# 1pathplanningzzj/pointnet_refine

Measured on AMD Instinct MI355X. Metric: lane segments/sec (fwd+bwd) at B=4096,N=1024; HBM GB/s vs roofline, higher is better.
Workload: dtype f32 (large GEMMs: 2xfp16-split MFMA, 3 products, fp32 accumulate); 1 GPU; LineRefineNet training step (fwd + deep-supervision L1 + bwd + Adam), B=4096/GPU, N=1024, M=32, C=4; global_batch=4096, points=1024, parallelism=dp1, decoder_chunk=4096

## Files before the change

include/pointnet_refine_hip.h:

```cpp
#ifndef POINTNET_REFINE_HIP_H
#define POINTNET_REFINE_HIP_H

#include <stddef.h>
#include <stdint.h>

#ifdef __cplusplus
extern "C" {
#endif

#define PRH_OK 0
#define PRH_ERR_ARG (-1)
#define PRH_ERR_WORKSPACE (-2)
#define PRH_ERR_HIP (-3)

#define PRH_MAX_LAYERS 8

typedef struct {
  const float* w;
  const float* b;
  const float* gamma;
  const float* beta;
  float* running_mean;
  float* running_var;
  int64_t* num_batches_tracked;
// ... 396 lines not shown
                         int device, void* stream);

int prh_set_gemm_mode(int mode);
int prh_get_gemm_mode(void);

int prh_set_dropout_seed_source(const unsigned* device_word);

int prh_test_gemm_nt(const float* a, const float* w, float* c, int m, int n, int k,
                     void* workspace, size_t workspace_bytes, int device, void* stream);
size_t prh_test_gemm_tn_workspace_bytes(int p, int mo, int ni);
size_t prh_test_gate_backward_workspace_bytes(int out_dim);
int prh_test_gate_backward(const float* ctx, int B, int N, int in_channel, int out_dim, const float* gate_w1,
                           const float* gate_b1, const float* gate_w2, const float* gate_b2, const float* z_fus,
                           const float* bn_scale, const float* bn_shift, float* d_fused, float* gate, int recompute,
                           float* ws_a, float* ws_b, void* workspace, size_t workspace_bytes, int device, void* stream);
int prh_test_gemm_tn(const float* a, const float* b, float* c, float* colsum, int p, int mo,
                     int ni, void* workspace, size_t workspace_bytes, int device, void* stream);
size_t prh_test_gemm_tn_side_workspace_bytes(int p, int mo, int ni);
int prh_test_gemm_tn_side(const float* a, const float* b, float* c, float* colsum, int p, int mo,
                          int ni, float* dy, long lddy, const float* z, long ldz, const float* ka,
                          const float* kb, const float* kc, long rows, int cols, int side,
                          float* amax_out, void* workspace, size_t workspace_bytes, int device,
                          void* stream);

enum {
  PRH_REDUCE_SLABS = 0, PRH_REDUCE_BN_STAGE1 = 1, PRH_REDUCE_PARTIALS = 2, PRH_REDUCE_LN_PARAM_GRAD = 3,
  PRH_REDUCE_FINAL = 4, PRH_REDUCE_ACT_AMAX = 5
};
int prh_test_reduce_depth(int kind);
int prh_test_reduce_slabs(const float* slab, int s, int rows, int cols, float* out, long ldout,
// ... 32 lines not shown
```

pointnet_refine_amd/_lib.py:

```python
from __future__ import annotations

import ctypes as C
import os
import subprocess
import threading

_HERE = os.path.dirname(os.path.abspath(__file__))
_ROOT = os.path.dirname(_HERE)
LIB_PATH = os.environ.get("PRH_LIB_PATH") or os.path.join(_HERE, "libpointnet_refine_hip.so")
_CSRC = os.path.join(_HERE, "csrc")
_SOURCES = [os.path.join(_CSRC, "prh_lib.hip")] + (sorted(
    os.path.join(_CSRC, f) for f in os.listdir(_CSRC) if f.endswith((".hpp", ".h", ".hip")) and f != "prh_lib.hip")
    if os.path.isdir(_CSRC) else [])
_HEADER = os.path.join(_ROOT, "include", "pointnet_refine_hip.h")

PRH_MAX_LAYERS = 8


class BnLayer(C.Structure):
    _fields_ = [("w", C.c_void_p), ("b", C.c_void_p), ("gamma", C.c_void_p), ("beta", C.c_void_p),
                ("running_mean", C.c_void_p), ("running_var", C.c_void_p),
                ("num_batches_tracked", C.c_void_p), ("cin", C.c_int), ("cout", C.c_int)]


# ... 30 lines not shown
    "prh_encoder_bf16_workspace_bytes", "prh_encoder_forward_bf16", "prh_encoder_backward_bf16",
    "prh_linear_bf16_workspace_bytes", "prh_linear_forward_bf16", "prh_linear_backward_bf16",
    "prh_linear_forward_out16", "prh_linear_backward_dy16", "prh_attn_forward_kv16", "prh_attn_backward_kv16",
    "prh_encoder_fused_image_bytes", "prh_encoder_fused_prepare", "prh_encoder_fused_workspace_bytes",
    "prh_encoder_fused_forward",
    "prh_linear_forward_workspace_bytes", "prh_linear_forward", "prh_linear_forward_ex",
    "prh_linear_forward_full", "prh_linear_forward_amax", "prh_operand_absmax_workspace_bytes", "prh_operand_absmax",
    "prh_linear_uses_operand_maxima", "prh_linear_backward_full", "prh_linear_backward_amax", "prh_pos_hidden_forward",
    "prh_pos_hidden_forward_workspace_bytes", "prh_pos_hidden_forward_amax", "prh_pos_hidden_backward_workspace_bytes",
    "prh_pos_hidden_backward", "prh_linear_small_forward", "prh_linear_small_backward_workspace_bytes",
    "prh_linear_small_backward",
    "prh_linear_backward_workspace_bytes", "prh_linear_backward", "prh_linear_backward_ex",
    "prh_mlp_stack_workspace_bytes", "prh_mlp_stack_forward", "prh_mlp_stack_backward",
    "prh_test_gemm_nt", "prh_test_gemm_tn_workspace_bytes", "prh_test_gemm_tn",
    "prh_test_gate_backward_workspace_bytes", "prh_test_gate_backward",
    "prh_test_gemm_tn_side_workspace_bytes", "prh_test_gemm_tn_side", "prh_test_xcc_map",
    "prh_test_reduce_depth", "prh_test_reduce_slabs", "prh_test_reduce_bn_stage1", "prh_test_reduce_partials",
    "prh_test_reduce_ln_param_grad", "prh_test_reduce_pos_hidden_final", "prh_test_reduce_partial_rows_final",
    "prh_test_reduce_act_amax_workspace_bytes", "prh_test_reduce_act_amax",
    "prh_profile_enable", "prh_profile_count", "prh_profile_reset", "prh_profile_read",
    "prh_attn_forward", "prh_attn_backward", "prh_attn_backward_ex",
    "prh_context_workspace_bytes", "prh_context_build",
    "prh_context_ragged_workspace_bytes", "prh_context_ragged_count", "prh_context_ragged_select",
    "prh_line_metrics", "prh_shift_sweep_workspace_bytes", "prh_shift_sweep",
    "prh_shift_sweep_ragged_workspace_bytes", "prh_shift_sweep_ragged",
    "prh_drive_slice_workspace_bytes", "prh_drive_slice_count", "prh_drive_slice_write",
    "prh_drive_clip_workspace_bytes", "prh_drive_clip_count", "prh_drive_clip_write",
    "prh_drive_noise_workspace_bytes", "prh_drive_noise",
    "prh_match_clip_workspace_bytes", "prh_match_clip_count", "prh_match_clip_write",
    "prh_match_costs_workspace_bytes", "prh_match_costs", "prh_match_max_side", "prh_match_assign",
# ... 329 lines not shown
    lib.prh_set_dropout_seed_source.argtypes = [vp]
    lib.prh_get_gemm_mode.restype = i
    lib.prh_profile_enable.restype = i
    lib.prh_profile_enable.argtypes = [i]
    lib.prh_profile_count.restype = i
    lib.prh_profile_reset.restype = i
    lib.prh_profile_read.restype = i
    lib.prh_profile_read.argtypes = [i, C.c_char_p, i, C.POINTER(C.c_float), C.POINTER(C.c_double),
                                     C.POINTER(C.c_double)]
    lib.prh_test_gemm_nt.restype = i
    lib.prh_test_gemm_nt.argtypes = [vp, vp, vp, i, i, i, vp, sz, i, vp]
    lib.prh_test_gate_backward_workspace_bytes.restype = sz
    lib.prh_test_gate_backward_workspace_bytes.argtypes = [i]
    lib.prh_test_gate_backward.restype = i
    lib.prh_test_gate_backward.argtypes = [vp, i, i, i, i, vp, vp, vp, vp, vp, vp, vp, vp, vp, i, vp, vp, vp, sz, i, vp]
    lib.prh_test_gemm_tn_workspace_bytes.restype = sz
    lib.prh_test_gemm_tn_workspace_bytes.argtypes = [i, i, i]
    lib.prh_test_gemm_tn.restype = i
    lib.prh_test_gemm_tn.argtypes = [vp, vp, vp, vp, i, i, i, vp, sz, i, vp]
    lib.prh_test_gemm_tn_side_workspace_bytes.restype = sz
    lib.prh_test_gemm_tn_side_workspace_bytes.argtypes = [i, i, i]
    lib.prh_test_gemm_tn_side.restype = i
    lib.prh_test_gemm_tn_side.argtypes = [vp, vp, vp, vp, i, i, i, vp, lg, vp, lg, vp, vp, vp, lg, i, i, vp, vp, sz, i, vp]
    lib.prh_test_xcc_map.restype = i
    lib.prh_test_xcc_map.argtypes = [i, i, vp, i, vp]
    if not hasattr(lib, "prh_test_reduce_depth"):
        return lib
    lib.prh_test_reduce_depth.restype = i
    lib.prh_test_reduce_depth.argtypes = [i]
    lib.prh_test_reduce_slabs.restype = i
# ... 38 lines not shown
```

pointnet_refine_amd/csrc/prh_gemm.hpp:

```cpp
#pragma once
#include <hip/hip_runtime.h>
#include <type_traits>
#include <stdint.h>

namespace prh {

typedef float f32x16 __attribute__((ext_vector_type(16)));

enum { PRO_NONE = 0, PRO_BNRELU = 1, PRO_BNBWD = 2, PRO_GATE1 = 3 };
enum { EPI_BIAS = 0, EPI_BIAS_STATS = 1, EPI_GATE = 2, EPI_DGRAD = 3, EPI_GATE_BWD = 4 };

enum {
  F_RELU_OUT = 1,
  F_ACCUM = 2,
  F_MASK = 4,
  F_STATS = 8,
  F_STORE_GATE = 16,
  F_E1_ROWVEC = 32,
  F_RESID = 64,
  F_DROPOUT = 256,
  F_POOL = 128,
};

struct NTParams {
  const float* A;  long lda;
  const float* A2; long lda2;
  const float* W;  long ldw;
  float* C;        long ldc;
  int M, N, K;
  const float* bias;
  const float* pa; const float* pb; const float* pc;
  const float* E1; long lde1;
  const float* es; const float* et;
  float* C2;       long ldc2;
  float* ws_a; float* ws_b;
  float* ws_c; float* ws_d;
  int flags;
  int tiles_n;
  char* wprep;
  const float* amaxA;
  const float* amaxW;
  unsigned drop_seed, drop_thresh;
  float drop_scale;
  const unsigned* seed_src;
};

__device__ __forceinline__ bool epi_keep(unsigned seed, unsigned row, unsigned col, unsigned thresh) {
  unsigned x = seed ^ (row * 0x9E3779B1u) ^ (col * 0x85EBCA77u);
  x ^= x >> 16; x *= 0x85EBCA6Bu; x ^= x >> 13; x *= 0xC2B2AE35u; x ^= x >> 16;
  return x >= thresh;
}
__device__ __forceinline__ unsigned epi_seed(const NTParams& p) {
  if (p.seed_src == nullptr) return p.drop_seed;
  const unsigned w = __hip_atomic_load(p.seed_src, __ATOMIC_RELAXED, __HIP_MEMORY_SCOPE_AGENT);
  return p.drop_seed ^ (__builtin_amdgcn_readfirstlane(w) * 0x9E3779B9u);
}

constexpr int BM = 128, BN = 128, BK = 32;

// ... 316 lines not shown
template <bool H>
__device__ __forceinline__ void st4e(char* base, int off, float4 v) {
  if (H) *reinterpret_cast<uint2*>(base + (size_t)off * 2) = make_uint2(pack_bf16x2(v.x, v.y), pack_bf16x2(v.z, v.w));
  else *reinterpret_cast<float4*>(base + (size_t)off * 4) = v;
}

typedef char* __restrict__ epi_wptr_r;
typedef const char* __restrict__ epi_rptr_r;
template <int EPI, int MT, class ACC, bool C16, bool AMAX = false>
__device__ __forceinline__ void nt_epilogue_vec_r2(ACC& acc, const NTParams& p, int rbase_,
                                                int cbase, int rb, int lane, float* scratch,
                                                bool bias_done = false,
                                                float* wave_amax = nullptr,
                                                float* zscr = nullptr) {
  static_assert(!AMAX || (EPI == EPI_BIAS && !C16), "output maximum: EPI_BIAS with fp32 storage");
  static_assert(EPI != EPI_GATE_BWD || !C16, "gate backward: fp32 storage");
  typedef typename std::conditional<AMAX || EPI == EPI_GATE_BWD, char*, epi_wptr_r>::type wptr;
  typedef typename std::conditional<AMAX || EPI == EPI_GATE_BWD, const char*, epi_rptr_r>::type rptr;
  const int rbase = __builtin_amdgcn_readfirstlane(rbase_);
  const float* biasp = bias_done ? nullptr : p.bias;
  constexpr int ES = C16 ? 2 : 4;
  const bool rowvec = EPI == EPI_DGRAD && (p.flags & F_E1_ROWVEC) != 0;
  const int ees = (C16 && !rowvec) ? 2 : 4;
  wptr Cb = reinterpret_cast<char*>(p.C) + (size_t)rbase * p.ldc * ES;
  rptr Eb = p.E1 != nullptr ? reinterpret_cast<const char*>(p.E1) + (size_t)rbase * p.lde1 * ees : nullptr;
  const int ldc = (int)p.ldc, lde1 = (int)p.lde1;
  const int mrows = p.M - rbase;
  const int rr = lane >> 4, c4 = (lane & 15) * 4;
  const int col4 = cbase + c4;
  const bool c4ok = col4 < p.N;
  float4 bias4 = zero4(), es4 = zero4(), et4 = zero4();
  if (c4ok) {
    if (biasp != nullptr) bias4 = ldg4(biasp + col4);
    if ((EPI == EPI_DGRAD && (p.flags & F_MASK) != 0) || EPI == EPI_GATE || EPI == EPI_GATE_BWD) {
      es4 = ldg4(p.es + col4);
      et4 = ldg4(p.et + col4);
    }
  }
  char* __restrict__ C2b = ((EPI == EPI_GATE || EPI == EPI_GATE_BWD) && p.C2 != nullptr) ? reinterpret_cast<char*>(p.C2) + (size_t)rbase * p.ldc2 * ES : nullptr;
  const int ldc2 = (int)p.ldc2;

  if (EPI == EPI_BIAS_STATS) epi_col_stats(acc, p, cbase, mrows, rb, lane, biasp);

  const bool mask = (p.flags & F_MASK) != 0, accum = (p.flags & F_ACCUM) != 0;
  const bool stats = EPI == EPI_DGRAD && (p.flags & F_STATS) != 0;
  const bool resid = EPI == EPI_BIAS && (p.flags & F_RESID) != 0;
  const unsigned dseed = (EPI == EPI_BIAS && (p.flags & F_DROPOUT) != 0) ? epi_seed(p) : 0u;
  const bool need_z = (EPI == EPI_DGRAD && (mask || stats)) || EPI == EPI_GATE || EPI == EPI_GATE_BWD || resid;
  float4 s1 = zero4(), s2 = zero4();
  const bool pool = EPI == EPI_GATE && (p.flags & F_POOL) != 0;
  float pmx[4] = {-1.f, -1.f, -1.f, -1.f}, psm[4] = {0.f, 0.f, 0.f, 0.f};
  int pix[4] = {0, 0, 0, 0};
  const int col4c = col4 < p.N ? col4 : (p.N - 4);
  rptr Cl = mrows > 0 ? Cb : reinterpret_cast<const char*>(p.C);
  rptr El = mrows > 0 ? Eb : reinterpret_cast<const char*>(p.E1);
  const bool acc_old = (EPI == EPI_DGRAD && accum) || EPI == EPI_GATE_BWD;
  float amx = 0.f;
  float t1 = 0.f, t2 = 0.f;
  constexpr int NB = 2 * MT;
  float4 zz[2][4], oo[2][4];
  auto issue = [&](int b, float4 (&z)[4], float4 (&o)[4]) {
    const char* Em = El; const char* Cm = Cl;
    asm volatile("" : "+s"(Em), "+s"(Cm) : : "memory");
    int lrc[4];
#pragma unroll
    for (int i = 0; i < 4; ++i) {
      z[i] = zero4(); o[i] = zero4();
      int r = (b >> 1) * 32 + ((b & 1) * 4 + i) * 4 + rr;
      r = r < mrows ? r : mrows - 1;
      lrc[i] = r < 0 ? 0 : r;
    }
// ... 57 lines not shown
          for (int e = 0; e < 4; ++e) {
            if (vv[e] > pmx[e]) { pmx[e] = vv[e]; pix[e] = lr; }
            psm[e] += vv[e];
          }
        }
      } else if (EPI == EPI_GATE_BWD) {
        const float4 m = gate_m4(v);
        float4 dg;
        gate_bwd_elem(o.x, z.x, m.x, es4.x, et4.x, v.x, dg.x);
        gate_bwd_elem(o.y, z.y, m.y, es4.y, et4.y, v.y, dg.y);
        gate_bwd_elem(o.z, z.z, m.z, es4.z, et4.z, v.z, dg.z);
        gate_bwd_elem(o.w, z.w, m.w, es4.w, et4.w, v.w, dg.w);
        if (ok) st4e<C16>(C2b, lr * ldc2 + col4, dg);
        *reinterpret_cast<float4*>(scratch + lrow * EPI_LDW + c4) = v;
        *reinterpret_cast<float4*>(zscr + (i * 4 + rr) * EPI_LDW + c4) = z;
      } else {
        if (resid) { v.x += z.x; v.y += z.y; v.z += z.z; v.w += z.w; }
        if ((p.flags & F_RELU_OUT) != 0) {
          v.x = fmaxf(v.x, 0.f); v.y = fmaxf(v.y, 0.f); v.z = fmaxf(v.z, 0.f); v.w = fmaxf(v.w, 0.f);
        }
        if (EPI == EPI_BIAS && (p.flags & F_DROPOUT) != 0) {
          const unsigned rw = (unsigned)(rbase + lr), c0 = (unsigned)col4;
          v.x = epi_keep(dseed, rw, c0, p.drop_thresh) ? v.x * p.drop_scale : 0.f;
          v.y = epi_keep(dseed, rw, c0 + 1, p.drop_thresh) ? v.y * p.drop_scale : 0.f;
          v.z = epi_keep(dseed, rw, c0 + 2, p.drop_thresh) ? v.z * p.drop_scale : 0.f;
          v.w = epi_keep(dseed, rw, c0 + 3, p.drop_thresh) ? v.w * p.drop_scale : 0.f;
        }
      }
      if (ok) st4e<C16>(Cb, lr * ldc + col4, v);
      if (AMAX && ok) amx = fmaxf(fmaxf(amx, fmaxf(fabsf(v.x), fabsf(v.y))), fmaxf(fabsf(v.z), fabsf(v.w)));
    }
    if (EPI == EPI_DGRAD)
      asm volatile("" : "+v"(s1.x), "+v"(s1.y), "+v"(s1.z), "+v"(s1.w), "+v"(s2.x), "+v"(s2.y), "+v"(s2.z), "+v"(s2.w));
    if constexpr (EPI == EPI_GATE_BWD) {
      const int nv = mrows - (mt * 32 + hb * 16);
      float c1 = 0.f, c2 = 0.f;
      if (nv >= 16) {
#pragma unroll
        for (int j = 0; j < 16; ++j) {
          const float dyj = scratch[(hb * 16 + j) * EPI_LDW + lane];
          c1 += dyj;
          c2 = fmaf(dyj, zscr[j * EPI_LDW + lane], c2);
        }
      } else {
        int nvv = nv;
// ... 31 lines not shown
      *reinterpret_cast<float4*>(p.ws_a + (size_t)rb * p.N + col4) = make_float4(pmx[0], pmx[1], pmx[2], pmx[3]);
      *reinterpret_cast<float4*>(p.ws_b + (size_t)rb * p.N + col4) = make_float4(psm[0], psm[1], psm[2], psm[3]);
      *reinterpret_cast<int4*>(p.ws_c + (size_t)rb * p.N + col4) = make_int4(pix[0], pix[1], pix[2], pix[3]);
    }
  }
  if (stats) {
    s1.x += __shfl_xor(s1.x, 16); s1.y += __shfl_xor(s1.y, 16); s1.z += __shfl_xor(s1.z, 16); s1.w += __shfl_xor(s1.w, 16);
    s2.x += __shfl_xor(s2.x, 16); s2.y += __shfl_xor(s2.y, 16); s2.z += __shfl_xor(s2.z, 16); s2.w += __shfl_xor(s2.w, 16);
    s1.x += __shfl_xor(s1.x, 32); s1.y += __shfl_xor(s1.y, 32); s1.z += __shfl_xor(s1.z, 32); s1.w += __shfl_xor(s1.w, 32);
    s2.x += __shfl_xor(s2.x, 32); s2.y += __shfl_xor(s2.y, 32); s2.z += __shfl_xor(s2.z, 32); s2.w += __shfl_xor(s2.w, 32);
    if (lane < 16 && c4ok) {
      *reinterpret_cast<float4*>(p.ws_a + (size_t)rb * p.N + col4) = s1;
      *reinterpret_cast<float4*>(p.ws_b + (size_t)rb * p.N + col4) = s2;
    }
  }
  if (AMAX) {
#pragma unroll
    for (int o = 32; o > 0; o >>= 1) amx = fmaxf(amx, __shfl_xor(amx, o));
    *wave_amax = amx;
  }
}

template <int EPI, int MT, class ACC, bool C16 = false, bool AMAX = false>
__device__ __forceinline__ void nt_epilogue_vec(ACC& acc, const NTParams& p, int rbase_,
                                                int cbase, int rb, int lane, float* scratch,
                                                bool bias_done = false,
                                                float* wave_amax = nullptr,
                                                float* zscr = nullptr) {
  if constexpr (!C16) {
    nt_epilogue_vec_r2<EPI, MT, ACC, false, AMAX>(acc, p, rbase_, cbase, rb, lane, scratch, bias_done, wave_amax, zscr);
    return;
  }
  static_assert(EPI != EPI_GATE_BWD || !C16, "gate backward: fp32 storage");
  const int rbase = __builtin_amdgcn_readfirstlane(rbase_);
  const float* biasp = bias_done ? nullptr : p.bias;
  constexpr int ES = C16 ? 2 : 4;
  const bool rowvec = EPI == EPI_DGRAD && (p.flags & F_E1_ROWVEC) != 0;
  const int ees = (C16 && !rowvec) ? 2 : 4;
  char* __restrict__ Cb = reinterpret_cast<char*>(p.C) + (size_t)rbase * p.ldc * ES;
  const char* __restrict__ Eb = p.E1 != nullptr ? reinterpret_cast<const char*>(p.E1) + (size_t)rbase * p.lde1 * ees : nullptr;
  const int ldc = (int)p.ldc, lde1 = (int)p.lde1;
  const int mrows = p.M - rbase;
  const int rr = lane >> 4, c4 = (lane & 15) * 4;
  const int col4 = cbase + c4;
  const bool c4ok = col4 < p.N;
  float4 bias4 = zero4(), es4 = zero4(), et4 = zero4();
  if (c4ok) {
    if (biasp != nullptr) bias4 = ldg4(biasp + col4);
// ... 424 lines not shown
```

pointnet_refine_amd/csrc/prh_gemm_h2.hpp:

```cpp
#pragma once
#include "prh_gemm_s3.hpp"

namespace prh {

constexpr int H2_BK = 32;
constexpr int H2_PLANE = 256 * H2_BK * 2;
constexpr int H2_OPER = 2 * H2_PLANE;
constexpr int H2_STAGE = 2 * H2_OPER;
constexpr int H2_LDS = 2 * H2_STAGE;

__device__ __forceinline__ int h2_off(int row, int k) {
  return row * 64 + ((((k >> 3) ^ (-(row >> 2))) & 3) << 4) + ((k & 7) << 1);
}

inline size_t h2_weight_bytes(int N, int K) {
  return S3_WHDR + (size_t)((N + 255) / 256) * ((K + H2_BK - 1) / H2_BK) * H2_OPER;
}

__global__ __launch_bounds__(256) void prep_weights_h2_kernel(const float* __restrict__ W, int N,
                                                              int K, long ldw, char* __restrict__ out,
                                                              const float* __restrict__ amax) {
  const int KT = (K + H2_BK - 1) / H2_BK;
  const int NT_ = (N + 255) / 256;
  const long total = (long)NT_ * 256 * KT * 4;
// ... 278 lines not shown
      tile(kt + 1, std::integral_constant<int, 0>{}, std::false_type{});
    }
    if (kt < KT) tile(kt, std::integral_constant<int, 1>{}, std::true_type{});
    if (kt + 1 < KT) tile(kt + 1, std::integral_constant<int, 0>{}, std::true_type{});
    if (wr == 0) __builtin_amdgcn_s_barrier();
  }
  asm volatile("s_waitcnt vmcnt(0)" ::: "memory");
  __syncthreads();
  PRH_TICK(1)
#pragma unroll
  for (int i = 0; i < 8; ++i)
#pragma unroll
    for (int j = 0; j < 4; ++j)
#pragma unroll
      for (int r = 0; r < 4; ++r) acc[i][j][r] *= unscale;
  if constexpr (AMAX) {
    float wmax = 0.f;
    nt_epilogue_vec<EPI, 4, f32x4[8][4], false, true>(acc, p, m0 + wm, n0 + wn, tile_m * 2 + (wave >> 2), lane,
                                                       reinterpret_cast<float*>(smem) + wave * (32 * EPI_LDW), false, &wmax);
    __syncthreads();
    float* red = reinterpret_cast<float*>(smem);
    if (lane == 0) red[wave] = wmax;
    __syncthreads();
    if (tid == 0)
      p.ws_a[blockIdx.x] = fmaxf(fmaxf(fmaxf(red[0], red[1]), fmaxf(red[2], red[3])),
                                 fmaxf(fmaxf(red[4], red[5]), fmaxf(red[6], red[7])));
  } else if constexpr (EPI == EPI_GATE_BWD) {
    static_assert(8 * (32 + 16) * EPI_LDW * 4 <= H2_LDS, "gate-backward scratch must fit in the stage buffers");
    nt_epilogue_vec<EPI, 4>(acc, p, m0 + wm, n0 + wn, tile_m * 2 + (wave >> 2), lane,
                            reinterpret_cast<float*>(smem) + wave * (32 * EPI_LDW), false, nullptr,
                            reinterpret_cast<float*>(smem) + 8 * (32 * EPI_LDW) + wave * (16 * EPI_LDW));
  } else {
    nt_epilogue_vec<EPI, 4>(acc, p, m0 + wm, n0 + wn, tile_m * 2 + (wave >> 2), lane,
// ... 309 lines not shown
```

pointnet_refine_amd/csrc/prh_lib.hip:

```cpp
#include "../../include/pointnet_refine_hip.h"

#include <hip/hip_runtime.h>
#include <stdarg.h>
#include <stdio.h>
#include <string.h>

#include <mutex>
#include <vector>

#include <stdlib.h>

#include "prh_gemm.hpp"
#include "prh_attn.hpp"
#include "prh_attn16.hpp"
#include "prh_gemm_s3.hpp"
#include "prh_gemm_h2.hpp"
#include "prh_b16.hpp"
#include "prh_small.hpp"
#include "prh_attnfold.hpp"
#include "prh_fused.hpp"
#include "prh_context.hpp"
#include "prh_metrics.hpp"
#include "prh_drive.hpp"
#include "prh_match.hpp"
// ... 385 lines not shown
}
template <int PRO, int EPI>
int launch_nt_core(Cores c, NTParams& p, hipStream_t st, StatInfo* si, float* amax_part, long* amax_tiles) {
  if (p.M <= 0 || p.N <= 0) return PRH_OK;
  if ((p.K & 3) || (PRO != PRO_GATE1 && (p.lda & 3)) || (p.ldw & 3) ||
      (PRO == PRO_BNBWD && (p.lda2 & 3)))
    return fail(PRH_ERR_ARG, "gemm_nt: K/lda/ldw must be multiples of 4 (K=%d lda=%ld ldw=%ld)",
                p.K, p.lda, p.ldw);
  if constexpr (PRO == PRO_NONE && EPI == EPI_BIAS) {
    if (c.mode == 4 && c.core == 2 && nt_b16_generic_ok(p)) return launch_nt_b16<PRO_NONE, EPI_BIAS, false, false>(p, st, si);
  }
  const bool want_pool = (p.flags & F_POOL) != 0;
  p.flags &= ~F_POOL;
  char nm[64];
  const double by = 4.0 * ((double)p.M * p.K * (PRO == PRO_BNBWD ? 2 : (PRO == PRO_GATE1 ? 0 : 1)) +
                           (double)p.M * p.N * (EPI == EPI_GATE_BWD ? 4 : (EPI == EPI_GATE ? 3 : (EPI == EPI_DGRAD ? 2 : 1))) +
                           (double)p.N * p.K);
  {
    if (p.wprep != nullptr && nt_use_s3(c, p.M, p.N, p.K) && p.lda <= 65536 && p.lda2 <= 65536 &&
        !((EPI == EPI_GATE || EPI == EPI_GATE_BWD) && ((p.N | (int)p.ldc | (int)p.lde1 | (int)p.ldc2) & 3) != 0)) {
      const int KT = cdiv(p.K, S3_BK), NTl = cdiv(p.N, S3_BN);
      const long th = (long)NTl * 256 * KT * 2;
      float* hdr = reinterpret_cast<float*>(p.wprep);
      const char* img = p.wprep + S3_WHDR;
      if (c.core == 3) {
        if (p.amaxW == nullptr) {
          TRY_RC((measure_absmax<PRO_NONE>(p.W, p.ldw, nullptr, 0, nullptr, nullptr, nullptr, p.N, p.K, hdr, hdr + 64, st)));
          p.amaxW = hdr;
        }
        if (p.amaxA == nullptr) {
          TRY_RC((measure_absmax<PRO>(p.A, p.lda, p.A2, p.lda2, p.pa, p.pb, p.pc, p.M, p.K, hdr + 1, hdr + 64, st)));
          p.amaxA = hdr + 1;
        }
      }
      if constexpr (PRO == PRO_NONE || PRO == PRO_BNRELU || PRO == PRO_GATE1) {
// ... 23 lines not shown
              *amax_tiles = wgs;
              return PRH_OK;
            }
          }
          if (g_h2_pp)
            hipLaunchKernelGGL((gemm_nt_h2_kernel<PRO, EPI, true>), dim3((unsigned)(NTl * cdiv(p.M, 256))), dim3(512),
                               lds, st, p, img);
          else
            hipLaunchKernelGGL((gemm_nt_h2_kernel<PRO, EPI>), dim3((unsigned)(NTl * cdiv(p.M, 256))), dim3(512),
                               lds, st, p, img);
          LAUNCH_CHECK();
          if (si) { si->count = 2 * cdiv(p.M, S3_BM); si->rows = 128; }
          return PRH_OK;
        }
      }
      if constexpr (EPI != EPI_GATE_BWD) {
        hipLaunchKernelGGL(prep_weights_s3_kernel, dim3((unsigned)cdiv(th, 256)), dim3(256), 0, st,
                           p.W, p.N, p.K, p.ldw, 0, p.wprep + S3_WHDR, c.core == 3 ? p.amaxW : nullptr);
        LAUNCH_CHECK();
        p.tiles_n = NTl;
        const long tiles = (long)NTl * cdiv(p.M, S3_BM);
        static const int attr_rc = allow_big_lds(gemm_nt_s3_kernel<PRO, EPI, 3>, gemm_nt_s3_kernel<PRO, EPI, 1>,
                                                 gemm_nt_s3_kernel<PRO, EPI, 2>);
        if (attr_rc != PRH_OK) return attr_rc;
        snprintf(nm, sizeof(nm), "gemm_nt_%s<%d,%d> K=%d N=%d", c.core == 3 ? "h2g1" : c.tag(), PRO, EPI, p.K, p.N);
        ProfScope ps(nm, 2.0 * p.M * (double)p.N * p.K, by, st);
        switch (c.core) {
          case 2: launch_nt_s3<PRO, EPI, 1>(p, tiles, img, st); break;
          case 3: launch_nt_s3<PRO, EPI, 2>(p, tiles, img, st); break;
          default: launch_nt_s3<PRO, EPI, 3>(p, tiles, img, st);
        }
        LAUNCH_CHECK();
        if (si) { si->count = 2 * cdiv(p.M, S3_BM); si->rows = 128; }
        return PRH_OK;
      }
    }
  }
  if constexpr (EPI == EPI_GATE_BWD) {
    return fail(PRH_ERR_ARG, "gemm_nt: the gate-recompute backward needs the split-fp16 core (M=%d N=%d)", p.M, p.N);
  } else {
    if constexpr (PRO == PRO_NONE && EPI == EPI_BIAS) {
      if (small_nt_ok(p, false)) return launch_small<false>(p, st);
    }
    p.tiles_n = cdiv(p.N, BN);
    const long tiles = (long)p.tiles_n * cdiv(p.M, BM);
    snprintf(nm, sizeof(nm), "gemm_nt<%d,%d> K=%d N=%d", PRO, EPI, p.K, p.N);
    ProfScope ps(nm, 2.0 * p.M * (double)p.N * p.K, by, st);
    if (p.N <= 64)
      hipLaunchKernelGGL((gemm_nt_kernel<PRO, EPI, true>), dim3((unsigned)tiles), dim3(256), 0, st, p);
    else
      hipLaunchKernelGGL((gemm_nt_kernel<PRO, EPI>), dim3((unsigned)tiles), dim3(256), 0, st, p);
    LAUNCH_CHECK();
    if (si) { si->count = 2 * cdiv(p.M, BM); si->rows = 64; }
// ... 991 lines not shown
  const int P = B * N;
  if (!recompute) {
    hipLaunchKernelGGL(combine_bwd_kernel, dim3(cdiv(P, 64), cdiv(od, 64)), dim3(256), 0, st, d_fused, d_gfeat,
                       argmax, z_fus, gate, es, et, P, N, od, dyf, ws_a, ws_b);
    LAUNCH_CHECK();
    return PRH_OK;
  }
  if (dyf != d_fused)
    HIP_TRY(hipMemcpyAsync(dyf, d_fused, (size_t)P * od * sizeof(float), hipMemcpyDeviceToDevice, st));
  NTParams p; memset(&p, 0, sizeof(p));
  p.A = inten; p.lda = C; p.pa = gate_w1; p.pb = gate_b1;
  p.W = gate_w2; p.ldw = 64; p.K = 64; p.M = P; p.N = od; p.bias = gate_b2;
  p.E1 = z_fus; p.lde1 = od; p.es = es; p.et = et;
  p.C = dyf; p.ldc = od; p.C2 = gate; p.ldc2 = od;
  p.ws_a = ws_a; p.ws_b = ws_b; p.wprep = wprep;
  return launch_nt<PRO_GATE1, EPI_GATE_BWD>(c, p, st);
}

int prh_encoder_gate_recompute(int B, int N, int in_channel, int out_dim, int want_global) {
  if (B <= 0 || N <= 0 || in_channel < 4 || out_dim <= 0 || (long)B * N > 2000000000L) return 0;
  return (!want_global && gate_on_h2(cores_of(gemm_mode()), B * N, out_dim, in_channel)) ? 1 : 0;
}

int prh_encoder_forward(const prh_encoder_params* prm, const float* ctx, int B, int N,
                        int training, float momentum, float eps, float* fused, float* gfeat,
                        const prh_encoder_saved* sv, void* workspace, size_t workspace_bytes,
                        int device, void* stream) {
  TRY(check_encoder(prm));
  if (!ctx || !fused || !sv || !sv->z_cat || !sv->z_fus || !sv->bn_scale || !sv->bn_shift ||
      !sv->bn_mean || !sv->bn_rstd || B <= 0 || N <= 0)
    return fail(PRH_ERR_ARG, "encoder_forward: bad argument");
// ... 79 lines not shown
  enc_carve(c, a, ews, P, prm->conv, cat, od, d_fused_scratch ? 2 : 1);
  StackWS& w = ews.w;
  StackBwdScratch& sc = ews.sc;
  float *fslab = ews.fslab, *fcslab = ews.fcslab, *dy_cat = ews.dy_cat, *dU = ews.dU, *dyf = d_fused_scratch ? d_fused : ews.dyf;
  float *gsum_a = ews.gsum_a, *gsum_b = ews.gsum_b;
  if (!a.ok) return fail(PRH_ERR_WORKSPACE, "encoder_backward: workspace too small (%zu bytes)", workspace_bytes);
  StackDims d = stack_dims(prm->conv, 5);
  if (d.cin0p != d.cin0) {
    TRY(copy_cols(ctx, d.cin0, d.cin0, w.xpad, d.cin0p, d.cin0p, (size_t)P, st));
    TRY(copy_cols(prm->conv[0].w, d.cin0, d.cin0, w.w0pad, d.cin0p, d.cin0p, (size_t)prm->conv[0].cout, st));
  }

  if (sv->gate_recompute && (d_gfeat != nullptr || !gate_on_h2(c, P, od, C)))
    return fail(PRH_ERR_ARG, "encoder_backward: saved.gate_recompute without prh_encoder_gate_recompute() "
                             "(pooled gradient, GEMM mode or shape)");
  TRY(gate_combine_backward(c, ctx + 3, C, B, N, od, prm->gate_w1, prm->gate_b1, prm->gate_w2, prm->gate_b2, sv->z_fus,
                            sv->bn_scale + cat, sv->bn_shift + cat, d_fused, d_gfeat, sv->argmax, sv->gate,
                            sv->gate_recompute, dyf, w.ws_a, w.ws_b, w.wprep, st));
  TRY(reduce_bn_stage1(w.ws_a, w.ws_b, cdiv(P, 64), (long)od, od, 64, P, 0, w.stat2, st));
  hipLaunchKernelGGL(bn_bwd_finalize_kernel, dim3(cdiv(od, 128)), dim3(128), 0, st, w.stat2, P, od,
                     prm->fusion.gamma, sv->bn_mean + cat, sv->bn_rstd + cat,
                     training, sc.ca, sc.cb, sc.cc, gr->fusion.dgamma, gr->fusion.dbeta,
                     gr->fusion.db);
  LAUNCH_CHECK();
  float* dG = sv->gate;

  StatInfo si5;
  const float* dzf_amax = nullptr;
  const bool matf = dz_in_place(c, od, (long)od, (long)od);
  if (matf) {
    TRY(materialize_dz(dyf, (long)od, sv->z_fus, (long)od, sc.ca, sc.cb, sc.cc, P, od, sc.hdr[0], st));
    dzf_amax = sc.hdr[0];
  }
  HeldWgrad hf;
  if (gr->fusion.dw) {
    TNParams t; memset(&t, 0, sizeof(t));
    t.A = dyf; t.lda = od; t.A2 = sv->z_fus; t.lda2 = od; t.pa = sc.ca; t.pb = sc.cb; t.pc = sc.cc;
    t.B = sv->z_cat; t.ldb = cat; t.qa = sv->bn_scale; t.qb = sv->bn_shift;
    t.P = P; t.Mo = od; t.Ni = cat;
    t.amaxA = dzf_amax;
    if (training && c.mode == 3 && sv->op_amax != nullptr) t.amaxB = sv->op_amax + 5;
    if (matf && dz_in_place(c, od, (long)cat, (long)cat) &&
        tn_side_ok(c, t, side_job(dy_cat + d.off[4], (long)cat, sv->z_cat + d.off[4], (long)cat, sc, P, od, sc.hdr[1]))) {
      hf.on = true; hf.t = t; hf.slab = fslab; hf.colslab = fcslab; hf.out = gr->fusion.dw; hf.ldc = (long)cat;
    } else if (matf) TRY((launch_tn<PRO_NONE, PRO_BNRELU>(c, t, fslab, fcslab, gr->fusion.dw, (long)cat, nullptr, st)));
// ... 1965 lines not shown
  p.A = a; p.lda = k; p.W = w; p.ldw = k; p.C = c; p.ldc = n; p.M = m; p.N = n; p.K = k;
  if (workspace != nullptr && workspace_bytes >= s3_weight_bytes(n, k) + 256)
    p.wprep = (char*)(((uintptr_t)workspace + 255) & ~(uintptr_t)255);
  return launch_nt<PRO_NONE, EPI_BIAS>(cores_of(gemm_mode()), p, (hipStream_t)stream);
}
size_t prh_test_gate_backward_workspace_bytes(int out_dim) { return s3_weight_bytes(out_dim, 64) + 512; }
int prh_test_gate_backward(const float* ctx, int B, int N, int in_channel, int out_dim, const float* gate_w1,
                           const float* gate_b1, const float* gate_w2, const float* gate_b2, const float* z_fus,
                           const float* bn_scale, const float* bn_shift, float* d_fused, float* gate, int recompute,
                           float* ws_a, float* ws_b, void* workspace, size_t workspace_bytes, int device, void* stream) {
  HIP_TRY(hipSetDevice(device));
  if (!ctx || !gate_w1 || !gate_b1 || !gate_w2 || !gate_b2 || !z_fus || !bn_scale || !bn_shift || !d_fused || !gate ||
      !ws_a || !ws_b || B <= 0 || N <= 0 || in_channel < 4 || out_dim <= 0 || (long)B * N > 2000000000L)
    return fail(PRH_ERR_ARG, "test_gate_backward: bad argument");
  const Cores c = cores_of(gemm_mode());
  if (recompute && !gate_on_h2(c, B * N, out_dim, in_channel))
    return fail(PRH_ERR_ARG, "test_gate_backward: recompute without prh_encoder_gate_recompute()");
  if (workspace == nullptr || workspace_bytes < prh_test_gate_backward_workspace_bytes(out_dim))
    return fail(PRH_ERR_WORKSPACE, "test_gate_backward: workspace too small");
  char* wprep = (char*)(((uintptr_t)workspace + 255) & ~(uintptr_t)255);
  return gate_combine_backward(c, ctx + 3, in_channel, B, N, out_dim, gate_w1, gate_b1, gate_w2, gate_b2, z_fus, bn_scale,
                               bn_shift, d_fused, nullptr, nullptr, gate, recompute, d_fused, ws_a, ws_b, wprep,
                               (hipStream_t)stream);
}
int prh_test_xcc_map(int blocks, int lds_bytes, int* out, int device, void* stream) {
  HIP_TRY(hipSetDevice(device));
  if (blocks <= 0 || lds_bytes < 0 || lds_bytes > 160 * 1024 || out == nullptr)
    return fail(PRH_ERR_ARG, "test_xcc_map: bad arguments");
  static const int attr_rc = allow_big_lds(xcc_probe_kernel);
  if (attr_rc != PRH_OK) return attr_rc;
  hipLaunchKernelGGL(xcc_probe_kernel, dim3((unsigned)blocks), dim3(512), (size_t)lds_bytes,
                     (hipStream_t)stream, out);
  LAUNCH_CHECK();
  return PRH_OK;
}
size_t prh_test_gemm_tn_workspace_bytes(int p, int mo, int ni) {
  const Cores c = cores_of(gemm_mode());
  Arena a;
// ... 119 lines not shown
```

pointnet_refine_amd/ops.py:

```python
from __future__ import annotations

import ctypes as C
import math
import threading
import weakref
from typing import List, Optional, Sequence

import torch

from . import _lib as L

_workspaces = {}


def _ws(device: torch.device, nbytes: int) -> torch.Tensor:
    key = (device.index, torch.cuda.current_stream(device).cuda_stream)
    t = _workspaces.get(key)
    if t is None or t.numel() < nbytes:
        _workspaces.pop(key, None)
        t = None
        t = torch.empty(int(nbytes * 1.05) + 4096, dtype=torch.uint8, device=device)
        _workspaces[key] = t
    return t

# ... 826 lines not shown
        elif ENCODER_RETAIN_GRAPH:
            gate = gate.clone()
        scratch = (d_fused is not None and d_gfeat is None and d_fused.is_contiguous() and not ENCODER_RETAIN_GRAPH
                   and d_fused.dtype == torch.float32
                   and (d_fused._base is None or d_fused._base.numel() == d_fused.numel()))
        if d_fused is not None:
            d_fused = d_fused.contiguous()
        if d_gfeat is not None:
            if not ctx.has_argmax:
                raise RuntimeError("encoder backward: gradient for global_feat but no argmax saved")
            d_gfeat = d_gfeat.contiguous()
        prm = _enc_params_struct(p2, None, Cin)
        same_mode = ctx.training and ctx.gemm_mode == L.lib().prh_get_gemm_mode()
        sv = L.EncoderSaved(_p(z_cat), _p(z_fus), _p(gate), _p(coef[0]), _p(coef[1]), _p(coef[2]),
                            _p(coef[3]), _p(argmax) if ctx.has_argmax else None,
                            _p(coef[4]) if same_mode else None, int(ctx.gate_recompute))
        gb = [_grad_buf(ctx.sinks[i], t.shape, dev) for i, t in enumerate(p2)]
        g = [b_[0] for b_ in gb]
        gr = L.EncoderGrads()
        for k in range(5):
            gr.conv[k] = L.BnLayerGrad(_p(g[2 * k]), _p(g[2 * k + 1]), _p(g[10 + 2 * k]), _p(g[11 + 2 * k]))
        gr.fusion = L.BnLayerGrad(_p(g[20]), _p(g[21]), _p(g[22]), _p(g[23]))
        gr.d_gate_w1, gr.d_gate_b1, gr.d_gate_w2, gr.d_gate_b2 = _p(g[24]), _p(g[25]), _p(g[26]), _p(g[27])
        dx = torch.empty_like(x) if ctx.needs_input_grad[0] else None
        nb = L.lib().prh_encoder_workspace_bytes(B, N, Cin, out_dim, 2 if scratch else 1)
        ws = _ws(dev, nb)
        L.check(L.lib().prh_encoder_backward(C.byref(prm), _p(x), B, N, ctx.training, _p(d_fused),
                                             _p(d_gfeat), int(scratch), C.byref(sv), C.byref(gr), _p(dx), _p(ws),
                                             ws.numel(), dev.index, _stream(dev)),
                "prh_encoder_backward")
        grads = [_grad_ret(*b_) for b_ in gb]
        grads = [gi.reshape(s) if gi is not None else None for gi, s in zip(grads, ctx.pshapes)]
        return (dx, None, None, None, None, None, *grads)


ENCODER_RETAIN_GRAPH = False
GATE_RECOMPUTE = True


def allow_encoder_retain_graph(flag: bool = True):
    global ENCODER_RETAIN_GRAPH
    ENCODER_RETAIN_GRAPH = bool(flag)


def encoder(x_pm, params, buffers, want_global: bool, training: bool, momentum: float, eps: float):
    return EncoderFn.apply(x_pm, want_global, training, momentum, eps, list(buffers), *params)


def encoder_with_amax(x_pm, params, buffers, want_global, training, momentum, eps):
    EncoderFn.last_fused_amax = None
    gfeat, fused = EncoderFn.apply(x_pm, want_global, training, momentum, eps, list(buffers), *params)
    amax, EncoderFn.last_fused_amax = EncoderFn.last_fused_amax, None
# ... 564 lines not shown
```

Measured before the change: 9972 segments/s.

## Recompute gate backward in a second GEMM pass to apply BN backward in epilogue

Result: no change. 10050 segments/s, median of 6 (+0.8%).

```diff
diff --git a/include/pointnet_refine_hip.h b/include/pointnet_refine_hip.h
--- a/include/pointnet_refine_hip.h
+++ b/include/pointnet_refine_hip.h
@@ -434,6 +434,12 @@
                            const float* gate_b1, const float* gate_w2, const float* gate_b2, const float* z_fus,
                            const float* bn_scale, const float* bn_shift, float* d_fused, float* gate, int recompute,
                            float* ws_a, float* ws_b, void* workspace, size_t workspace_bytes, int device, void* stream);
+size_t prh_test_gate_dz_workspace_bytes(int P, int out_dim);
+int prh_test_gate_dz(const float* ctx, int B, int N, int in_channel, int out_dim, const float* gate_w1,
+                     const float* gate_b1, const float* gate_w2, const float* gate_b2, const float* z_fus,
+                     const float* bn_scale, const float* bn_shift, const float* gamma, const float* bn_mean,
+                     const float* bn_rstd, float* d_fused, float* gate, int mode, float* ws_a, float* ws_b,
+                     float* coef, float* amax, void* workspace, size_t workspace_bytes, int device, void* stream);
 int prh_test_gemm_tn(const float* a, const float* b, float* c, float* colsum, int p, int mo,
                      int ni, void* workspace, size_t workspace_bytes, int device, void* stream);
 size_t prh_test_gemm_tn_side_workspace_bytes(int p, int mo, int ni);
diff --git a/pointnet_refine_amd/_lib.py b/pointnet_refine_amd/_lib.py
--- a/pointnet_refine_amd/_lib.py
+++ b/pointnet_refine_amd/_lib.py
@@ -68,6 +68,7 @@
     "prh_mlp_stack_workspace_bytes", "prh_mlp_stack_forward", "prh_mlp_stack_backward",
     "prh_test_gemm_nt", "prh_test_gemm_tn_workspace_bytes", "prh_test_gemm_tn",
     "prh_test_gate_backward_workspace_bytes", "prh_test_gate_backward",
+    "prh_test_gate_dz_workspace_bytes", "prh_test_gate_dz",
     "prh_test_gemm_tn_side_workspace_bytes", "prh_test_gemm_tn_side", "prh_test_xcc_map",
     "prh_test_reduce_depth", "prh_test_reduce_slabs", "prh_test_reduce_bn_stage1", "prh_test_reduce_partials",
     "prh_test_reduce_ln_param_grad", "prh_test_reduce_pos_hidden_final", "prh_test_reduce_partial_rows_final",
@@ -427,6 +428,10 @@
     lib.prh_test_gate_backward_workspace_bytes.argtypes = [i]
     lib.prh_test_gate_backward.restype = i
     lib.prh_test_gate_backward.argtypes = [vp, i, i, i, i, vp, vp, vp, vp, vp, vp, vp, vp, vp, i, vp, vp, vp, sz, i, vp]
+    lib.prh_test_gate_dz_workspace_bytes.restype = sz
+    lib.prh_test_gate_dz_workspace_bytes.argtypes = [i, i]
+    lib.prh_test_gate_dz.restype = i
+    lib.prh_test_gate_dz.argtypes = [vp, i, i, i, i] + [vp] * 12 + [i, vp, vp, vp, vp, vp, sz, i, vp]
     lib.prh_test_gemm_tn_workspace_bytes.restype = sz
     lib.prh_test_gemm_tn_workspace_bytes.argtypes = [i, i, i]
     lib.prh_test_gemm_tn.restype = i
diff --git a/pointnet_refine_amd/csrc/prh_gemm.hpp b/pointnet_refine_amd/csrc/prh_gemm.hpp
--- a/pointnet_refine_amd/csrc/prh_gemm.hpp
+++ b/pointnet_refine_amd/csrc/prh_gemm.hpp
@@ -8,7 +8,7 @@
 typedef float f32x16 __attribute__((ext_vector_type(16)));
 
 enum { PRO_NONE = 0, PRO_BNRELU = 1, PRO_BNBWD = 2, PRO_GATE1 = 3 };
-enum { EPI_BIAS = 0, EPI_BIAS_STATS = 1, EPI_GATE = 2, EPI_DGRAD = 3, EPI_GATE_BWD = 4 };
+enum { EPI_BIAS = 0, EPI_BIAS_STATS = 1, EPI_GATE = 2, EPI_DGRAD = 3, EPI_GATE_BWD = 4, EPI_GATE_DZ = 5 };
 
 enum {
   F_RELU_OUT = 1,
@@ -20,6 +20,7 @@
   F_RESID = 64,
   F_DROPOUT = 256,
   F_POOL = 128,
+  F_KEEP_C = 512,
 };
 
 struct NTParams {
@@ -43,6 +44,7 @@
   unsigned drop_seed, drop_thresh;
   float drop_scale;
   const unsigned* seed_src;
+  const float* ka; const float* kb; const float* kc;
 };
 
 __device__ __forceinline__ bool epi_keep(unsigned seed, unsigned row, unsigned col, unsigned thresh) {
@@ -389,9 +391,11 @@
                                                 float* wave_amax = nullptr,
                                                 float* zscr = nullptr) {
   static_assert(!AMAX || (EPI == EPI_BIAS && !C16), "output maximum: EPI_BIAS with fp32 storage");
-  static_assert(EPI != EPI_GATE_BWD || !C16, "gate backward: fp32 storage");
-  typedef typename std::conditional<AMAX || EPI == EPI_GATE_BWD, char*, epi_wptr_r>::type wptr;
-  typedef typename std::conditional<AMAX || EPI == EPI_GATE_BWD, const char*, epi_rptr_r>::type rptr;
+  static_assert((EPI != EPI_GATE_BWD && EPI != EPI_GATE_DZ) || !C16, "gate backward: fp32 storage");
+  constexpr bool GATE_B = EPI == EPI_GATE_BWD || EPI == EPI_GATE_DZ;
+  constexpr bool VMAX = AMAX || EPI == EPI_GATE_DZ;
+  typedef typename std::conditional<AMAX || GATE_B, char*, epi_wptr_r>::type wptr;
+  typedef typename std::conditional<AMAX || GATE_B, const char*, epi_rptr_r>::type rptr;
   const int rbase = __builtin_amdgcn_readfirstlane(rbase_);
   const float* biasp = bias_done ? nullptr : p.bias;
   constexpr int ES = C16 ? 2 : 4;
@@ -407,11 +411,14 @@
   float4 bias4 = zero4(), es4 = zero4(), et4 = zero4();
   if (c4ok) {
     if (biasp != nullptr) bias4 = ldg4(biasp + col4);
-    if ((EPI == EPI_DGRAD && (p.flags & F_MASK) != 0) || EPI == EPI_GATE || EPI == EPI_GATE_BWD) {
+    if ((EPI == EPI_DGRAD && (p.flags & F_MASK) != 0) || EPI == EPI_GATE || GATE_B) {
       es4 = ldg4(p.es + col4);
       et4 = ldg4(p.et + col4);
     }
   }
+  float4 ka4 = zero4(), kb4 = zero4(), kc4 = zero4();
+  if (EPI == EPI_GATE_DZ && c4ok) { ka4 = ldg4(p.ka + col4); kb4 = ldg4(p.kb + col4); kc4 = ldg4(p.kc + col4); }
+  const bool keep_c = EPI == EPI_GATE_BWD && (p.flags & F_KEEP_C) != 0;
   char* __restrict__ C2b = ((EPI == EPI_GATE || EPI == EPI_GATE_BWD) && p.C2 != nullptr) ? reinterpret_cast<char*>(p.C2) + (size_t)rbase * p.ldc2 * ES : nullptr;
   const int ldc2 = (int)p.ldc2;
 
@@ -421,7 +428,7 @@
   const bool stats = EPI == EPI_DGRAD && (p.flags & F_STATS) != 0;
   const bool resid = EPI == EPI_BIAS && (p.flags & F_RESID) != 0;
   const unsigned dseed = (EPI == EPI_BIAS && (p.flags & F_DROPOUT) != 0) ? epi_seed(p) : 0u;
-  const bool need_z = (EPI == EPI_DGRAD && (mask || stats)) || EPI == EPI_GATE || EPI == EPI_GATE_BWD || resid;
+  const bool need_z = (EPI == EPI_DGRAD && (mask || stats)) || EPI == EPI_GATE || GATE_B || resid;
   float4 s1 = zero4(), s2 = zero4();
   const bool pool = EPI == EPI_GATE && (p.flags & F_POOL) != 0;
   float pmx[4] = {-1.f, -1.f, -1.f, -1.f}, psm[4] = {0.f, 0.f, 0.f, 0.f};
@@ -429,7 +436,7 @@
   const int col4c = col4 < p.N ? col4 : (p.N - 4);
   rptr Cl = mrows > 0 ? Cb : reinterpret_cast<const char*>(p.C);
   rptr El = mrows > 0 ? Eb : reinterpret_cast<const char*>(p.E1);
-  const bool acc_old = (EPI == EPI_DGRAD && accum) || EPI == EPI_GATE_BWD;
+  const bool acc_old = (EPI == EPI_DGRAD && accum) || GATE_B;
   float amx = 0.f;
   float t1 = 0.f, t2 = 0.f;
   constexpr int NB = 2 * MT;
@@ -517,6 +524,14 @@
         if (ok) st4e<C16>(C2b, lr * ldc2 + col4, dg);
         *reinterpret_cast<float4*>(scratch + lrow * EPI_LDW + c4) = v;
         *reinterpret_cast<float4*>(zscr + (i * 4 + rr) * EPI_LDW + c4) = z;
+      } else if (EPI == EPI_GATE_DZ) {
+        const float4 m = gate_m4(v);
+        float4 dy, dg;
+        gate_bwd_elem(o.x, z.x, m.x, es4.x, et4.x, dy.x, dg.x);
+        gate_bwd_elem(o.y, z.y, m.y, es4.y, et4.y, dy.y, dg.y);
+        gate_bwd_elem(o.z, z.z, m.z, es4.z, et4.z, dy.z, dg.z);
+        gate_bwd_elem(o.w, z.w, m.w, es4.w, et4.w, dy.w, dg.w);
+        v = pro_apply<PRO_BNBWD>(dy, z, ka4, kb4, kc4);
       } else {
         if (resid) { v.x += z.x; v.y += z.y; v.z += z.z; v.w += z.w; }
         if ((p.flags & F_RELU_OUT) != 0) {
@@ -530,8 +545,8 @@
           v.w = epi_keep(dseed, rw, c0 + 3, p.drop_thresh) ? v.w * p.drop_scale : 0.f;
         }
       }
-      if (ok) st4e<C16>(Cb, lr * ldc + col4, v);
-      if (AMAX && ok) amx = fmaxf(fmaxf(amx, fmaxf(fabsf(v.x), fabsf(v.y))), fmaxf(fabsf(v.z), fabsf(v.w)));
+      if (ok && !keep_c) st4e<C16>(Cb, lr * ldc + col4, v);
+      if (VMAX && ok) amx = fmaxf(fmaxf(amx, fmaxf(fabsf(v.x), fabsf(v.y))), fmaxf(fabsf(v.z), fabsf(v.w)));
     }
     if (EPI == EPI_DGRAD)
       asm volatile("" : "+v"(s1.x), "+v"(s1.y), "+v"(s1.z), "+v"(s1.w), "+v"(s2.x), "+v"(s2.y), "+v"(s2.z), "+v"(s2.w));
@@ -593,7 +608,7 @@
       *reinterpret_cast<float4*>(p.ws_b + (size_t)rb * p.N + col4) = s2;
     }
   }
-  if (AMAX) {
+  if (VMAX) {
 #pragma unroll
     for (int o = 32; o > 0; o >>= 1) amx = fmaxf(amx, __shfl_xor(amx, o));
     *wave_amax = amx;
@@ -610,7 +625,7 @@
     nt_epilogue_vec_r2<EPI, MT, ACC, false, AMAX>(acc, p, rbase_, cbase, rb, lane, scratch, bias_done, wave_amax, zscr);
     return;
   }
-  static_assert(EPI != EPI_GATE_BWD || !C16, "gate backward: fp32 storage");
+  static_assert((EPI != EPI_GATE_BWD && EPI != EPI_GATE_DZ) || !C16, "gate backward: fp32 storage");
   const int rbase = __builtin_amdgcn_readfirstlane(rbase_);
   const float* biasp = bias_done ? nullptr : p.bias;
   constexpr int ES = C16 ? 2 : 4;
diff --git a/pointnet_refine_amd/csrc/prh_gemm_h2.hpp b/pointnet_refine_amd/csrc/prh_gemm_h2.hpp
--- a/pointnet_refine_amd/csrc/prh_gemm_h2.hpp
+++ b/pointnet_refine_amd/csrc/prh_gemm_h2.hpp
@@ -316,9 +316,9 @@
     for (int j = 0; j < 4; ++j)
 #pragma unroll
       for (int r = 0; r < 4; ++r) acc[i][j][r] *= unscale;
-  if constexpr (AMAX) {
+  if constexpr (AMAX || EPI == EPI_GATE_DZ) {
     float wmax = 0.f;
-    nt_epilogue_vec<EPI, 4, f32x4[8][4], false, true>(acc, p, m0 + wm, n0 + wn, tile_m * 2 + (wave >> 2), lane,
+    nt_epilogue_vec<EPI, 4, f32x4[8][4], false, AMAX>(acc, p, m0 + wm, n0 + wn, tile_m * 2 + (wave >> 2), lane,
                                                        reinterpret_cast<float*>(smem) + wave * (32 * EPI_LDW), false, &wmax);
     __syncthreads();
     float* red = reinterpret_cast<float*>(smem);
diff --git a/pointnet_refine_amd/csrc/prh_lib.hip b/pointnet_refine_amd/csrc/prh_lib.hip
--- a/pointnet_refine_amd/csrc/prh_lib.hip
+++ b/pointnet_refine_amd/csrc/prh_lib.hip
@@ -423,11 +423,12 @@
   p.flags &= ~F_POOL;
   char nm[64];
   const double by = 4.0 * ((double)p.M * p.K * (PRO == PRO_BNBWD ? 2 : (PRO == PRO_GATE1 ? 0 : 1)) +
-                           (double)p.M * p.N * (EPI == EPI_GATE_BWD ? 4 : (EPI == EPI_GATE ? 3 : (EPI == EPI_DGRAD ? 2 : 1))) +
+                           (double)p.M * p.N * (EPI == EPI_GATE_BWD ? ((p.flags & F_KEEP_C) != 0 ? 3 : 4) :
+                                               (EPI == EPI_GATE || EPI == EPI_GATE_DZ ? 3 : (EPI == EPI_DGRAD ? 2 : 1))) +
                            (double)p.N * p.K);
   {
     if (p.wprep != nullptr && nt_use_s3(c, p.M, p.N, p.K) && p.lda <= 65536 && p.lda2 <= 65536 &&
-        !((EPI == EPI_GATE || EPI == EPI_GATE_BWD) && ((p.N | (int)p.ldc | (int)p.lde1 | (int)p.ldc2) & 3) != 0)) {
+        !((EPI == EPI_GATE || EPI == EPI_GATE_BWD || EPI == EPI_GATE_DZ) && ((p.N | (int)p.ldc | (int)p.lde1 | (int)p.ldc2) & 3) != 0)) {
       const int KT = cdiv(p.K, S3_BK), NTl = cdiv(p.N, S3_BN);
       const long th = (long)NTl * 256 * KT * 2;
       float* hdr = reinterpret_cast<float*>(p.wprep);
@@ -481,7 +482,7 @@
           return PRH_OK;
         }
       }
-      if constexpr (EPI != EPI_GATE_BWD) {
+      if constexpr (EPI != EPI_GATE_BWD && EPI != EPI_GATE_DZ) {
         hipLaunchKernelGGL(prep_weights_s3_kernel, dim3((unsigned)cdiv(th, 256)), dim3(256), 0, st,
                            p.W, p.N, p.K, p.ldw, 0, p.wprep + S3_WHDR, c.core == 3 ? p.amaxW : nullptr);
         LAUNCH_CHECK();
@@ -503,7 +504,7 @@
       }
     }
   }
-  if constexpr (EPI == EPI_GATE_BWD) {
+  if constexpr (EPI == EPI_GATE_BWD || EPI == EPI_GATE_DZ) {
     return fail(PRH_ERR_ARG, "gemm_nt: the gate-recompute backward needs the split-fp16 core (M=%d N=%d)", p.M, p.N);
   } else {
     if constexpr (PRO == PRO_NONE && EPI == EPI_BIAS) {
@@ -1525,7 +1526,25 @@
   p.E1 = z_fus; p.lde1 = od; p.es = es; p.et = et;
   p.C = dyf; p.ldc = od; p.C2 = gate; p.ldc2 = od;
   p.ws_a = ws_a; p.ws_b = ws_b; p.wprep = wprep;
+  if (recompute == 2) p.flags = F_KEEP_C;
   return launch_nt<PRO_GATE1, EPI_GATE_BWD>(c, p, st);
+}
+int gate_dz_apply(Cores c, const float* inten, int C, int P, int od, const float* gate_w1, const float* gate_b1,
+                  const float* gate_w2, const float* gate_b2, const float* z_fus, const float* es, const float* et,
+                  const float* ka, const float* kb, const float* kc, float* dyf, float* part, float* amax,
+                  char* wprep, hipStream_t st) {
+  NTParams p; memset(&p, 0, sizeof(p));
+  p.A = inten; p.lda = C; p.pa = gate_w1; p.pb = gate_b1;
+  p.W = gate_w2; p.ldw = 64; p.K = 64; p.M = P; p.N = od; p.bias = gate_b2;
+  p.E1 = z_fus; p.lde1 = od; p.es = es; p.et = et;
+  p.ka = ka; p.kb = kb; p.kc = kc;
+  p.C = dyf; p.ldc = od;
+  p.ws_a = part; p.wprep = wprep;
+  TRY_RC((launch_nt<PRO_GATE1, EPI_GATE_DZ>(c, p, st)));
+  hipLaunchKernelGGL(absmax_final_kernel, dim3(1), dim3(256), 0, st, (const float*)part,
+                     cdiv(P, S3_BM) * cdiv(od, S3_BN), amax);
+  LAUNCH_CHECK();
+  return PRH_OK;
 }
 
 int prh_encoder_gate_recompute(int B, int N, int in_channel, int out_dim, int want_global) {
@@ -1635,6 +1654,8 @@
   if (sv->gate_recompute && (d_gfeat != nullptr || !gate_on_h2(c, P, od, C)))
     return fail(PRH_ERR_ARG, "encoder_backward: saved.gate_recompute without prh_encoder_gate_recompute() "
                              "(pooled gradient, GEMM mode or shape)");
+  if (sv->gate_recompute < 0 || sv->gate_recompute > 2)
+    return fail(PRH_ERR_ARG, "encoder_backward: saved.gate_recompute is 0, 1 or 2");
   TRY(gate_combine_backward(c, ctx + 3, C, B, N, od, prm->gate_w1, prm->gate_b1, prm->gate_w2, prm->gate_b2, sv->z_fus,
                             sv->bn_scale + cat, sv->bn_shift + cat, d_fused, d_gfeat, sv->argmax, sv->gate,
                             sv->gate_recompute, dyf, w.ws_a, w.ws_b, w.wprep, st));
@@ -1649,7 +1670,11 @@
   StatInfo si5;
   const float* dzf_amax = nullptr;
   const bool matf = dz_in_place(c, od, (long)od, (long)od);
-  if (matf) {
+  if (sv->gate_recompute == 2) {
+    TRY(gate_dz_apply(c, ctx + 3, C, P, od, prm->gate_w1, prm->gate_b1, prm->gate_w2, prm->gate_b2, sv->z_fus,
+                      sv->bn_scale + cat, sv->bn_shift + cat, sc.ca, sc.cb, sc.cc, dyf, w.ws_a, sc.hdr[0], w.wprep, st));
+    dzf_amax = sc.hdr[0];
+  } else if (matf) {
     TRY(materialize_dz(dyf, (long)od, sv->z_fus, (long)od, sc.ca, sc.cb, sc.cc, P, od, sc.hdr[0], st));
     dzf_amax = sc.hdr[0];
   }
@@ -3645,6 +3670,7 @@
       !ws_a || !ws_b || B <= 0 || N <= 0 || in_channel < 4 || out_dim <= 0 || (long)B * N > 2000000000L)
     return fail(PRH_ERR_ARG, "test_gate_backward: bad argument");
   const Cores c = cores_of(gemm_mode());
+  if (recompute < 0 || recompute > 2) return fail(PRH_ERR_ARG, "test_gate_backward: recompute is 0, 1 or 2");
   if (recompute && !gate_on_h2(c, B * N, out_dim, in_channel))
     return fail(PRH_ERR_ARG, "test_gate_backward: recompute without prh_encoder_gate_recompute()");
   if (workspace == nullptr || workspace_bytes < prh_test_gate_backward_workspace_bytes(out_dim))
@@ -3653,6 +3679,56 @@
   return gate_combine_backward(c, ctx + 3, in_channel, B, N, out_dim, gate_w1, gate_b1, gate_w2, gate_b2, z_fus, bn_scale,
                                bn_shift, d_fused, nullptr, nullptr, gate, recompute, d_fused, ws_a, ws_b, wprep,
                                (hipStream_t)stream);
+}
+struct GateDzWS { char* wprep; double* stat2; float* hdr; float* part; };
+static void gate_dz_carve(Arena& a, GateDzWS& w, int P, int od) {
+  w.wprep = (char*)a.f(s3_weight_bytes(od, 64) / sizeof(float) + 64);
+  w.stat2 = (double*)a.f((size_t)BN_SLICES * 3 * od * 2);
+  w.hdr = a.f(S3_HDR_FLOATS);
+  w.part = a.f(nt_amax_part_floats(P, od));
+}
+size_t prh_test_gate_dz_workspace_bytes(int P, int out_dim) {
+  if (P <= 0 || out_dim <= 0) return 0;
+  Arena a; GateDzWS w;
+  gate_dz_carve(a, w, P, out_dim);
+  return a.off + 256;
+}
+int prh_test_gate_dz(const float* ctx, int B, int N, int in_channel, int out_dim, const float* gate_w1,
+                     const float* gate_b1, const float* gate_w2, const float* gate_b2, const float* z_fus,
+                     const float* bn_scale, const float* bn_shift, const float* gamma, const float* bn_mean,
+                     const float* bn_rstd, float* d_fused, float* gate, int mode, float* ws_a, float* ws_b,
+                     float* coef, float* amax, void* workspace, size_t workspace_bytes, int device, void* stream) {
+  HIP_TRY(hipSetDevice(device));
+  if (!ctx || !gate_w1 || !gate_b1 || !gate_w2 || !gate_b2 || !z_fus || !bn_scale || !bn_shift || !gamma || !bn_mean ||
+      !bn_rstd || !d_fused || !gate || !ws_a || !ws_b || !coef || !amax || B <= 0 || N <= 0 || in_channel < 4 ||
+      out_dim <= 0 || (long)B * N > 2000000000L || mode < 0 || mode > 2)
+    return fail(PRH_ERR_ARG, "test_gate_dz: bad argument");
+  const Cores c = cores_of(gemm_mode());
+  const int P = B * N, od = out_dim;
+  if (mode != 0 && !gate_on_h2(c, P, od, in_channel))
+    return fail(PRH_ERR_ARG, "test_gate_dz: recompute without prh_encoder_gate_recompute()");
+  if (!dz_in_place(c, od, (long)od, (long)od))
+    return fail(PRH_ERR_ARG, "test_gate_dz: dz_f is materialised on the split-fp16 cores with out_dim %% 4 == 0 only");
+  hipStream_t st = (hipStream_t)stream;
+  Arena a(workspace, workspace_bytes);
+  GateDzWS w;
+  gate_dz_carve(a, w, P, od);
+  if (workspace == nullptr || !a.ok) return fail(PRH_ERR_WORKSPACE, "test_gate_dz: workspace too small");
+  float *ca = coef, *cb = coef + od, *cc = coef + 2 * (size_t)od;
+  TRY(gate_combine_backward(c, ctx + 3, in_channel, B, N, od, gate_w1, gate_b1, gate_w2, gate_b2, z_fus, bn_scale,
+                            bn_shift, d_fused, nullptr, nullptr, gate, mode, d_fused, ws_a, ws_b, w.wprep, st));
+  TRY(reduce_bn_stage1(ws_a, ws_b, cdiv(P, 64), (long)od, od, 64, P, 0, w.stat2, st));
+  hipLaunchKernelGGL(bn_bwd_finalize_kernel, dim3(cdiv(od, 128)), dim3(128), 0, st, w.stat2, P, od, gamma, bn_mean,
+                     bn_rstd, 1, ca, cb, cc, (float*)nullptr, (float*)nullptr, (float*)nullptr);
+  LAUNCH_CHECK();
+  if (mode == 2) {
+    TRY(gate_dz_apply(c, ctx + 3, in_channel, P, od, gate_w1, gate_b1, gate_w2, gate_b2, z_fus, bn_scale, bn_shift, ca,
+                      cb, cc, d_fused, w.part, w.hdr, w.wprep, st));
+  } else {
+    TRY(materialize_dz(d_fused, (long)od, z_fus, (long)od, ca, cb, cc, P, od, w.hdr, st));
+  }
+  HIP_TRY(hipMemcpyAsync(amax, w.hdr, sizeof(float), hipMemcpyDeviceToDevice, st));
+  return PRH_OK;
 }
 int prh_test_xcc_map(int blocks, int lds_bytes, int* out, int device, void* stream) {
   HIP_TRY(hipSetDevice(device));
diff --git a/pointnet_refine_amd/ops.py b/pointnet_refine_amd/ops.py
--- a/pointnet_refine_amd/ops.py
+++ b/pointnet_refine_amd/ops.py
@@ -864,7 +864,8 @@
         same_mode = ctx.training and ctx.gemm_mode == L.lib().prh_get_gemm_mode()
         sv = L.EncoderSaved(_p(z_cat), _p(z_fus), _p(gate), _p(coef[0]), _p(coef[1]), _p(coef[2]),
                             _p(coef[3]), _p(argmax) if ctx.has_argmax else None,
-                            _p(coef[4]) if same_mode else None, int(ctx.gate_recompute))
+                            _p(coef[4]) if same_mode else None,
+                            (2 if GATE_DZ_RECOMPUTE else 1) if ctx.gate_recompute else 0)
         gb = [_grad_buf(ctx.sinks[i], t.shape, dev) for i, t in enumerate(p2)]
         g = [b_[0] for b_ in gb]
         gr = L.EncoderGrads()
@@ -886,6 +887,7 @@
 
 ENCODER_RETAIN_GRAPH = False
 GATE_RECOMPUTE = True
+GATE_DZ_RECOMPUTE = True
 
 
 def allow_encoder_retain_graph(flag: bool = True):
```
